# ai4ce/DiscoNet

Measured on AMD Instinct MI355X. Metric: scenes/sec (5-agent 256x256 BEV), higher is better.
Workload: dtype f16 hi+lo pair per value (32 bits; 22-bit significand for |x| >= 0.125, f16 exponent range, lo subnormal below: absolute floor 2^-25); conv products as split-f16 x3 MFMA, f32 accumulate; 1 GPU; DiscoNet det eval forward (--com disco), 5-agent, batch 4 per GPU, 256x256x13 BEV, no KD, sparse voxel lists -> dense -> enc -> DiscoGraph fusion -> dec -> cls/reg heads; agents=5, batch_per_gpu=4, conv_math=sp, launch=hipGraph replay, parallelism=scene-parallel x1 (no data-path collective)

## Files before the change

disconet_amd/csrc/common.hip:

```cpp
#include "dn_internal.h"

namespace dn {
char* err_buf() {
  static thread_local char buf[512] = {0};
  return buf;
}
namespace {
typedef unsigned u32x4 __attribute__((ext_vector_type(4)));
__global__ void __launch_bounds__(256) zero_fill_kernel(unsigned char* p, size_t head, size_t vecs, size_t tail) {
  const size_t tid = blockIdx.x * (size_t)blockDim.x + threadIdx.x, stride = (size_t)gridDim.x * blockDim.x;
  if (tid < head) p[tid] = 0;
  u32x4* v = reinterpret_cast<u32x4*>(p + head);
  for (size_t i = tid; i < vecs; i += stride) v[i] = u32x4{0u, 0u, 0u, 0u};
  if (tid < tail) p[head + 16 * vecs + tid] = 0;
}
}

hipError_t zero_fill(void* ptr, size_t bytes, hipStream_t stream) {
  if (bytes == 0) return hipSuccess;
  unsigned char* p = static_cast<unsigned char*>(ptr);
  size_t head = (16 - (reinterpret_cast<size_t>(p) & 15)) & 15;
  if (head > bytes) head = bytes;
  const size_t vecs = (bytes - head) / 16, tail = bytes - head - 16 * vecs;
  const size_t want = (vecs + 255) / 256;
  const int blocks = (int)(want < 1 ? 1 : (want > 8192 ? 8192 : want));
  hipLaunchKernelGGL(zero_fill_kernel, dim3(blocks), dim3(256), 0, stream, p, head, vecs, tail);
  return hipGetLastError();
}
}

extern "C" int dn_version(void) { return 154; }

#ifndef DN_BUILD_ID
#error "build through disconet_amd/csrc/build.py (it passes -DDN_BUILD_ID)"
#endif
static const char dn_build_id_marker[] = "dn-build-id:" DN_BUILD_ID;
extern "C" const char* dn_build_id(void) { return dn_build_id_marker + 12; }

extern "C" int dn_sp_range_flags_async(unsigned* dst_device, int reset, void* stream) {
  DN_REQUIRE(dst_device != nullptr, "sp_range_flags_async: null destination");
  hipStream_t s = (hipStream_t)stream;
  if ((reset & 2) && dn::zero_fill(dst_device, sizeof(unsigned), s) != hipSuccess)
    return dn::fail(DN_ERR_LAUNCH, "sp_range_flags_async: zero fill of the destination failed");
  const bool clear = (reset & 1) != 0;
  dn::range_collect_conv_sp(dst_device, clear, s);
  dn::range_collect_conv_spq(dst_device, clear, s);
  dn::range_collect_fuse_mlp(dst_device, clear, s);
  dn::range_collect_conv_wgrad(dst_device, clear, s);
  return dn::check_launch("sp_range_collect_kernel");
}

extern "C" unsigned dn_sp_range_flags(int reset) {
  unsigned* d = nullptr;
  unsigned v = 0;
  if (hipDeviceSynchronize() != hipSuccess || hipMalloc((void**)&d, sizeof v) != hipSuccess) return 0x80000000u;
  bool ok = hipMemcpy(d, &v, sizeof v, hipMemcpyHostToDevice) == hipSuccess &&
            dn_sp_range_flags_async(d, reset ? 1 : 0, nullptr) == DN_OK &&
            hipMemcpy(&v, d, sizeof v, hipMemcpyDeviceToHost) == hipSuccess;
  (void)hipFree(d);
  return ok ? v : 0x80000000u;
}

extern "C" const char* dn_last_error(void) { return dn::err_buf(); }
```

disconet_amd/csrc/conv_spq.hip:

```cpp
#ifndef DN_SP_ABL
#define DN_SP_ABL 0
#endif
#include "dn_internal.h"
#include "sp_layout.h"
#include "sp_device.h"
#include "sp_split.h"
#include <type_traits>

namespace {

constexpr int kCUs = 256;

constexpr int QTH = 8, QTW = 32, QPH = QTH + 2, QPW = QTW + 2, QHALF = QPW / 2, QPITCH = QPW, QNPIX = QPH * QPITCH;
constexpr int QNW = 4, QNT = QNW * 64;
constexpr int QA_PIECES = 4 * QNPIX;
constexpr int QA_INSTR = (QA_PIECES + 63) / 64;
constexpr int QA_IT = (QA_INSTR + QNW - 1) / QNW;
constexpr int QA_STAGE = QA_INSTR * 1024;
static_assert(QA_INSTR == 22 && QA_IT == 6, "patch stage: 22 instructions, waves 0 / 1 issue 6, waves 2 / 3 issue 5");

struct SpqArgs {
  const unsigned char* src0;
  const unsigned char* src1;
  const unsigned char* wpk;
  const float* scale;
  const float* shift;
  unsigned char* out;
  float* out_f32;
  int ldo_f32;
  int n_images, h, w;
  int c0g, c1g;
  int c_out, cog, relu;
  int tiles_x, tiles_y, total_items;
  int cout_pad, wpk_bytes;
  int n_cb;
  float rcp_ncb, rcp_tx, rcp_ty;
  KSlices ks;
};

struct QTile {
  int img, oy0, ox0, n0;
};

template <int BN, int DEEP = 0>
struct SpqTile {
  static constexpr int WTN = BN / 32;
  static constexpr int TGQ = DEEP ? 4 : (BN == 64 ? 1 : 2);
  static constexpr int NS0 = 4 / TGQ;
  static constexpr int TG1 = DEEP ? 9 : 3;
  static constexpr int NS1 = 9 / TG1;
  static constexpr int BLK = 4 * BN * 16;
  static constexpr int B_PIECES0 = TGQ * 4 * 4 * BN;
  static constexpr int B_PIECES1 = TG1 * 4 * BN;
  static constexpr int B_IT0 = (B_PIECES0 + QNT - 1) / QNT;
  static constexpr int B_IT1 = (B_PIECES1 + QNT - 1) / QNT;
  static_assert(B_IT1 <= B_IT0, "the source-0 step is the larger one");
  static constexpr int QB_STAGE = B_IT0 * QNT * 16;
  static constexpr int AFF_BYTES = QNW * 2 * 64 * 4;
  static constexpr int LDS_BYTES = 2 * QA_STAGE + 2 * QB_STAGE + AFF_BYTES;
  static_assert((DEEP ? 1 : 2) * LDS_BYTES <= 160 * 1024, "two workgroups per CU (DEEP: one)");
};

template <int BN, int DEEP, int ABL = 0, int KSL = 0>
__global__ void __launch_bounds__(QNT, 2) conv_spq_kernel(const SpqArgs a) {
  static_assert(!KSL || BN == 32, "K slices: the 32-channel tile");
  using T = SpqTile<BN, DEEP>;
  constexpr int WTN = T::WTN, TGQ = T::TGQ, NS0 = T::NS0, NS1 = T::NS1, BLK = T::BLK, QB_STAGE = T::QB_STAGE;
  extern __shared__ __attribute__((aligned(16))) unsigned char smem[];
  constexpr int OFF_B = 2 * QA_STAGE;

  const int tid = threadIdx.x;
  const int lane = tid & 63;
  const int wave = tid >> 6;
  const int li = lane & 31, lh = lane >> 5;
  const int py = wave & 1, px = wave >> 1;

  const int G = gridDim.x;
  const int spatial_items = a.n_images * a.tiles_y * a.tiles_x;
  const int n_cb = a.n_cb;
  const int sp_full = spatial_items & ~7;
  auto decode = [&](int item) {
    QTile tc;
    int cb, spi;
    if (item < sp_full * n_cb) {
      const int j = item >> 3;
      const int jq = fdivmod(j, n_cb, a.rcp_ncb, cb);
      spi = (item & 7) * (sp_full >> 3) + jq;
    } else {
      const int r = item - sp_full * n_cb, rem = spatial_items - sp_full;
      cb = r / rem;
      spi = sp_full + r % rem;
    }
    tc.n0 = cb * BN;
    int tx, ty;
    spi = fdivmod(spi, a.tiles_x, a.rcp_tx, tx);
    tc.img = fdivmod(spi, a.tiles_y, a.rcp_ty, ty);
    tc.ox0 = tx * QTW;
    tc.oy0 = ty * QTH;
    return tc;
  };

  struct Work {
    QTile tc;
    int sl0, sl1, j;
  };
  const int nchunks = a.c0g + a.c1g;
  auto decode_work = [&](int v) {
    Work w;
    if (KSL == 0 || v < a.ks.n_whole) {
      w.tc = decode(v);
      w.sl0 = 0; w.sl1 = KSL ? a.ks.count : 1; w.j = -1;
    } else {
      w.j = v - a.ks.n_whole;
      w.sl0 = w.j & ((1 << a.ks.log2) - 1);
      w.sl1 = w.sl0 + 1;
      w.tc = decode(a.ks.n_whole + (w.j >> a.ks.log2));
    }
    return w;
  };
  auto first_group = [&](const Work& w) { return KSL ? a.ks.bound(w.sl0) : 0; };

  const int rsel = sp::in_g2(li) ? 1 : 0, kcol = sp::rank16(li);
  int prow[2], pcol;
  pcol = px + 2 * kcol;
  auto colpos = [](int e) { return (e & 1) * QHALF + (e >> 1); };
  int a_b1[2][3];
  int a_b0[2][2][2];
#pragma unroll
  for (int wm = 0; wm < 2; ++wm) {
    prow[wm] = py + 4 * wm + 2 * rsel;
#pragma unroll
    for (int dx = 0; dx < 3; ++dx) a_b1[wm][dx] = (lh * QNPIX + prow[wm] * QPITCH + colpos(px + dx) + kcol) * 16;
#pragma unroll
    for (int b = 0; b < 2; ++b)
#pragma unroll
      for (int am = 0; am < 2; ++am)
        a_b0[wm][b][am] = (lh * QNPIX + (prow[wm] + am + (py & am)) * QPITCH + colpos(px + b + (px & b)) + kcol) * 16;
  }
  int b_off[WTN], b_offq[WTN];
#pragma unroll
  for (int wn = 0; wn < WTN; ++wn) {
    b_off[wn] = (lh * BN + wn * 32 + li) * 16;
    b_offq[wn] = b_off[wn] + wave * BLK;
  }

  f32x16 acc[2][WTN];
  f32x16 tot[KSL ? 2 : 1][KSL ? WTN : 1];
  float amax = 0.f;
  bool nan_seen = false;

  constexpr unsigned OOB = 0xFFFFFFFFu;
  const int hs0 = a.h >> 1, ws0 = a.w >> 1;
  const unsigned plane0 = (unsigned)(hs0 * ws0) * 16u, plane1 = (unsigned)(a.h * a.w) * 16u;
  const size_t img0_bytes = (size_t)a.c0g * 4 * plane0, img1_bytes = (size_t)a.c1g * 4 * plane1;
  auto rsrc0 = __builtin_amdgcn_make_buffer_rsrc(const_cast<unsigned char*>(a.src0), 0, 0, 0x00020000);
  auto rsrc1 = rsrc0;
  const auto rsrcw = __builtin_amdgcn_make_buffer_rsrc(const_cast<unsigned char*>(a.wpk), 0, a.wpk_bytes, 0x00020000);
  unsigned voff_a[QA_IT], voff_b[T::B_IT0];

  auto opaque = [](int v) {
    asm volatile("" : "+v"(v));
    return v;
  };
  unsigned piece_map[QA_IT];
#pragma unroll
  for (int it = 0; it < QA_IT; ++it) {
    const int piece = (it * QNW + wave) * 64 + lane;
    const int cq = piece / QNPIX, pp = piece % QNPIX;
    const int r = pp / QPITCH, pos = pp % QPITCH;
    const int cc = pos < QHALF ? 2 * pos : 2 * (pos - QHALF) + 1;
    piece_map[it] = (unsigned)r | ((unsigned)cc << 8) | ((unsigned)cq << 16) | (piece < QA_PIECES ? 0x80000000u : 0u);
  }
  auto setup_voff_a = [&](const QTile& tc, bool from1) {
    const int iy0 = tc.oy0 - 1, ix0 = tc.ox0 - 1;
    const unsigned plane = from1 ? plane1 : plane0;
    const int ws = from1 ? a.w : ws0;
#pragma unroll
    for (int it = 0; it < QA_IT; ++it) {
      unsigned pm = piece_map[it];
      asm volatile("" : "+v"(pm));
      const int r = pm & 0xff, cc = (pm >> 8) & 0xff, cq = (pm >> 16) & 0xff;
      const int iy = iy0 + r, ix = ix0 + cc;
      const bool ok = (int)pm < 0 && iy >= 0 && iy < a.h && ix >= 0 && ix < a.w;
      const int sy = from1 ? iy : (iy >> 1), sx = from1 ? ix : (ix >> 1);
      voff_a[it] = ok ? (unsigned)cq * plane + (unsigned)(sy * ws + sx) * 16u : OOB;
    }
  };
  int voffb_n0 = -1;
  auto setup_voff_b = [&](const QTile& tc) {
    if (tc.n0 == voffb_n0) return;
    voffb_n0 = tc.n0;
    const int t = opaque(tid);
#pragma unroll
    for (int it = 0; it < T::B_IT0; ++it) {
      const int piece = (it * QNW + (t >> 6)) * 64 + (t & 63);
      const int blk = piece / (4 * BN), q = (piece / BN) % 4, nn = piece % BN;
      voff_b[it] = (unsigned)(((blk * 4 + q) * a.cout_pad + tc.n0 + nn) * 16);
    }
  };
  auto setup_rsrc = [&](const QTile& tc) {
    rsrc0 = __builtin_amdgcn_make_buffer_rsrc(const_cast<unsigned char*>(a.src0 + tc.img * img0_bytes), 0,
                                              (int)img0_bytes, 0x00020000);
    rsrc1 = __builtin_amdgcn_make_buffer_rsrc(const_cast<unsigned char*>(a.c1g ? a.src1 + tc.img * img1_bytes : a.src0),
                                              0, a.c1g ? (int)img1_bytes : 0, 0x00020000);
  };
  auto issue_a = [&](int g, int sa) {
    if constexpr ((ABL & 2) != 0) return;
    const bool from1 = g >= a.c0g;
    const int soff = from1 ? (g - a.c0g) * 4 * (int)plane1 : g * 4 * (int)plane0;
    unsigned char* base = smem + sa * QA_STAGE + wave * 1024;
#pragma unroll
    for (int it = 0; it < QA_IT; ++it) {
      if (it == QA_IT - 1 && wave >= QA_INSTR - (QA_IT - 1) * QNW) break;
      if (from1)
        dma16(rsrc1, base + it * QNW * 1024, voff_a[it], soff);
      else
        dma16(rsrc0, base + it * QNW * 1024, voff_a[it], soff);
    }
  };
  auto issue_b = [&](int g, int st, int sb) {
    if constexpr ((ABL & 1) != 0) return;
    const bool from1 = g >= a.c0g;
    const int blk = from1 ? a.c0g * 16 + (g - a.c0g) * 9 + st * T::TG1 : g * 16 + st * (TGQ * 4);
    const int soff = blk * 4 * a.cout_pad * 16;
    unsigned char* base = smem + OFF_B + sb * QB_STAGE + wave * 1024;
#pragma unroll
    for (int it = 0; it < T::B_IT0; ++it)
      if (!from1 || it < T::B_IT1) dma16(rsrcw, base + it * QNW * 1024, voff_b[it], soff);
  };

  struct Frags {
    half8 ah[2], al[2], bh[WTN], bl[WTN];
  };
  auto mma = [&](const Frags& f) {
#pragma unroll
    for (int wm = 0; wm < 2; ++wm)
#pragma unroll
      for (int k = 0; k < WTN; ++k) {
        const int wn = (wm & 1) ? WTN - 1 - k : k;
        acc[wm][wn] = __builtin_amdgcn_mfma_f32_32x32x16_f16(f.bl[wn], f.ah[wm], acc[wm][wn], 0, 0, 0);
      }
#pragma unroll
    for (int wm = 0; wm < 2; ++wm)
#pragma unroll
      for (int k = 0; k < WTN; ++k) {
        const int wn = (wm & 1) ? WTN - 1 - k : k;
        acc[wm][wn] = __builtin_amdgcn_mfma_f32_32x32x16_f16(f.bh[wn], f.al[wm], acc[wm][wn], 0, 0, 0);
      }
#pragma unroll
    for (int wm = 0; wm < 2; ++wm)
#pragma unroll
      for (int k = 0; k < WTN; ++k) {
        const int wn = (wm & 1) ? WTN - 1 - k : k;
        acc[wm][wn] = __builtin_amdgcn_mfma_f32_32x32x16_f16(f.bh[wn], f.ah[wm], acc[wm][wn], 0, 0, 0);
      }
  };
  auto compute1 = [&](auto st_c, const unsigned char* As, const unsigned char* Bs) {
    constexpr int DY = decltype(st_c)::value;
    Frags f[2];
    auto load = [&](auto u_c) {
      constexpr int u = decltype(u_c)::value;
      Frags& d = f[u & 1];
#pragma unroll
      for (int wm = 0; wm < 2; ++wm) {
        d.ah[wm] = *reinterpret_cast<const half8*>(As + a_b1[wm][u] + DY * QPITCH * 16);
        d.al[wm] = *reinterpret_cast<const half8*>(As + a_b1[wm][u] + DY * QPITCH * 16 + 2 * QNPIX * 16);
      }
#pragma unroll
      for (int wn = 0; wn < WTN; ++wn) {
        d.bh[wn] = *reinterpret_cast<const half8*>(Bs + b_off[wn] + u * BLK);
        d.bl[wn] = *reinterpret_cast<const half8*>(Bs + b_off[wn] + u * BLK + 2 * BN * 16);
      }
    };
    load(std::integral_constant<int, 0>{});
    load(std::integral_constant<int, 1>{});
    __builtin_amdgcn_sched_barrier(0);
    mma(f[0]);
    __builtin_amdgcn_sched_barrier(0);
    load(std::integral_constant<int, 2>{});
    __builtin_amdgcn_sched_barrier(0);
    mma(f[1]);
    __builtin_amdgcn_sched_barrier(0);
    mma(f[0]);
    __builtin_amdgcn_sched_barrier(0);
  };
  auto compute0 = [&](auto st_c, const unsigned char* As, const unsigned char* Bs) {
    constexpr int ST = decltype(st_c)::value;
    Frags f[2];
    auto load = [&](auto u_c) {
      constexpr int u = decltype(u_c)::value;
      constexpr int t = ST * TGQ + u, am = t >> 1, b = t & 1;
      Frags& d = f[u & 1];
#pragma unroll
      for (int wm = 0; wm < 2; ++wm) {
        d.ah[wm] = *reinterpret_cast<const half8*>(As + a_b0[wm][b][am]);
        d.al[wm] = *reinterpret_cast<const half8*>(As + a_b0[wm][b][am] + 2 * QNPIX * 16);
      }
#pragma unroll
      for (int wn = 0; wn < WTN; ++wn) {
        d.bh[wn] = *reinterpret_cast<const half8*>(Bs + b_offq[wn] + u * 4 * BLK);
        d.bl[wn] = *reinterpret_cast<const half8*>(Bs + b_offq[wn] + u * 4 * BLK + 2 * BN * 16);
      }
    };
    load(std::integral_constant<int, 0>{});
    if constexpr (TGQ == 4) {
      load(std::integral_constant<int, 1>{});
      __builtin_amdgcn_sched_barrier(0);
      mma(f[0]);
      __builtin_amdgcn_sched_barrier(0);
      load(std::integral_constant<int, 2>{});
      __builtin_amdgcn_sched_barrier(0);
      mma(f[1]);
      __builtin_amdgcn_sched_barrier(0);
      load(std::integral_constant<int, 3>{});
      __builtin_amdgcn_sched_barrier(0);
      mma(f[0]);
      __builtin_amdgcn_sched_barrier(0);
      mma(f[1]);
    } else if constexpr (TGQ == 2) {
      load(std::integral_constant<int, 1>{});
      __builtin_amdgcn_sched_barrier(0);
      mma(f[0]);
      __builtin_amdgcn_sched_barrier(0);
      mma(f[1]);
    } else {
      __builtin_amdgcn_sched_barrier(0);
      mma(f[0]);
    }
    __builtin_amdgcn_sched_barrier(0);
  };

  float* aff_s = reinterpret_cast<float*>(smem + 2 * QA_STAGE + 2 * QB_STAGE) + wave * 128;
  int aff_n0 = -1;
  auto load_affine = [&](int n0) {
    if (n0 == aff_n0) return;
    aff_n0 = n0;
    if (lane < BN) {
      const int co = n0 + lane, ci = min(co, a.c_out - 1);
      aff_s[lane] = co < a.c_out ? a.scale[ci] : 0.f;
      aff_s[64 + lane] = co < a.c_out ? a.shift[ci] : 0.f;
    }
  };
  auto epilogue = [&](const QTile& tc) {
    const int plane = a.h * a.w * 16;
    const int img_bytes = a.cog * 4 * plane;
    const auto rsrc_o = __builtin_amdgcn_make_buffer_rsrc(a.out + (size_t)tc.img * img_bytes, 0, img_bytes, 0x00020000);
    const float lo_clamp = a.relu ? 0.f : -65504.f;
    if (a.out_f32 != nullptr) {
      const float floor_v = a.relu ? 0.f : -__builtin_inff();
#pragma unroll
      for (int wm = 0; wm < 2; ++wm) {
        const int oy = tc.oy0 + prow[wm], ox = tc.ox0 + pcol;
        const bool inside = oy < a.h && ox < a.w;
        float* orow = a.out_f32 + (((size_t)tc.img * a.h + oy) * a.w + ox) * a.ldo_f32;
#pragma unroll
        for (int wn = 0; wn < WTN; ++wn)
#pragma unroll
          for (int g = 0; g < 4; ++g) {
            const int co = tc.n0 + 32 * wn + 8 * g + 4 * lh;
            const f32x4 sc = *reinterpret_cast<const f32x4*>(aff_s + wn * 32 + 8 * g + 4 * lh);
            const f32x4 sh = *reinterpret_cast<const f32x4*>(aff_s + 64 + wn * 32 + 8 * g + 4 * lh);
            f32x4 v = affine4(quad_of(acc[wm][wn], g), sc, sh);
            nan_seen |= !(fabsf(v[0]) <= 3.4028235e38f) | !(fabsf(v[1]) <= 3.4028235e38f) | !(fabsf(v[2]) <= 3.4028235e38f) |
                        !(fabsf(v[3]) <= 3.4028235e38f);
#pragma unroll
            for (int e = 0; e < 4; ++e) v[e] = fmaxf(v[e], floor_v);
            if (inside && co < a.c_out) *reinterpret_cast<f32x4*>(orow + co) = v;
          }
      }
      if (a.out == nullptr) return;
    }
#pragma unroll
    for (int wm = 0; wm < 2; ++wm) {
      const int oy = tc.oy0 + prow[wm], ox = tc.ox0 + pcol;
      const bool inside = oy < a.h && ox < a.w;
      const int voff = inside ? (oy * a.w + ox) * 16 + lh * plane : (int)0x80000000;
#pragma unroll
      for (int wn = 0; wn < WTN; ++wn) {
        u32x2 hi[4], lo[4];
#pragma unroll
        for (int g = 0; g < 4; ++g) {
          const f32x4 sc = *reinterpret_cast<const f32x4*>(aff_s + wn * 32 + 8 * g + 4 * lh);
          const f32x4 sh = *reinterpret_cast<const f32x4*>(aff_s + 64 + wn * 32 + 8 * g + 4 * lh);
          const f32x4 v = affine4(quad_of(acc[wm][wn], g), sc, sh);
          split4(v, hi[g], lo[g], amax, lo_clamp);
        }
#pragma unroll
        for (int m = 0; m < 2; ++m) {
          const u32x4 ph = gather_octet(hi[2 * m], hi[2 * m + 1]);
          const u32x4 pl = gather_octet(lo[2 * m], lo[2 * m + 1]);
          const int cg = (tc.n0 + 32 * wn) / 16 + m;
          if (cg < a.cog) {
            __builtin_amdgcn_raw_buffer_store_b128(ph, rsrc_o, voff + cg * 4 * plane, 0, 0);
            __builtin_amdgcn_raw_buffer_store_b128(pl, rsrc_o, voff + (cg * 4 + 2) * plane, 0, 0);
          }
        }
      }
    }
  };

  int item = blockIdx.x;
  if (item >= a.total_items) return;
  auto partial_of = [&](int j) {
    return a.ks.partial + ((size_t)j * QNW + wave) * (2 * WTN * 16 * 64) + lane * 4;
  };
  auto fold_acc = [&]() {
    if constexpr (KSL != 0) {
#pragma unroll
      for (int wm = 0; wm < 2; ++wm)
#pragma unroll
        for (int wn = 0; wn < WTN; ++wn)
#pragma unroll
          for (int r = 0; r < 16; ++r) {
            tot[wm][wn][r] += acc[wm][wn][r];
            acc[wm][wn][r] = 0.f;
          }
    }
  };
  auto zero_tot = [&]() {
    if constexpr (KSL != 0) {
#pragma unroll
      for (int wm = 0; wm < 2; ++wm)
#pragma unroll
        for (int wn = 0; wn < WTN; ++wn)
#pragma unroll
          for (int r = 0; r < 16; ++r) tot[wm][wn][r] = 0.f;
    }
  };
  auto tot_to_acc = [&]() {
    if constexpr (KSL != 0) {
#pragma unroll
      for (int wm = 0; wm < 2; ++wm)
#pragma unroll
        for (int wn = 0; wn < WTN; ++wn) acc[wm][wn] = tot[wm][wn];
    }
  };
  if constexpr (KSL != 0) {
    if (a.ks.fixup) {
      for (int p = blockIdx.x; p < a.ks.n_split; p += G) {
        const QTile tc = decode(a.ks.n_whole + p);
        load_affine(tc.n0);
        zero_tot();
        for (int sl = 0; sl < a.ks.count; ++sl) {
          const float* pb = partial_of((p << a.ks.log2) + sl);
#pragma unroll
          for (int wm = 0; wm < 2; ++wm)
#pragma unroll
            for (int wn = 0; wn < WTN; ++wn)
#pragma unroll
              for (int q = 0; q < 4; ++q) {
                const f32x4 v = *reinterpret_cast<const f32x4*>(pb + ((wm * WTN + wn) * 4 + q) * 256);
#pragma unroll
                for (int e = 0; e < 4; ++e) acc[wm][wn][4 * q + e] = v[e];
              }
          fold_acc();
        }
        tot_to_acc();
        epilogue(tc);
        note_range(amax, nan_seen);
      }
      return;
    }
  }
  Work cw = decode_work(item);
  QTile cur = cw.tc;
  setup_rsrc(cur);
  setup_voff_b(cur);
  setup_voff_a(cur, first_group(cw) >= a.c0g);
  issue_b(first_group(cw), 0, 0);
  issue_a(first_group(cw), 0);
  int sa = 0, sb = 0;
  bool a_pending = true;

  while (true) {
#pragma unroll
    for (int wm = 0; wm < 2; ++wm)
#pragma unroll
      for (int wn = 0; wn < WTN; ++wn)
#pragma unroll
        for (int r = 0; r < 16; ++r) acc[wm][wn][r] = 0.f;
    load_affine(cur.n0);
    const bool has_next = item + G < a.total_items;
    QTile nxt = cur;
    int ng0 = 0;
    if (has_next) {
      const Work nw = decode_work(item + G);
      nxt = nw.tc;
      ng0 = first_group(nw);
    }
    if constexpr (KSL != 0) zero_tot();
    const int g_end = KSL ? a.ks.bound(cw.sl1) : nchunks;

    for (int sl = cw.sl0; sl < cw.sl1; ++sl) {
    const int g_lo = KSL ? a.ks.bound(sl) : 0, g_hi = KSL ? a.ks.bound(sl + 1) : nchunks;
    for (int g = g_lo; g < g_hi; ++g) {
      const bool last_g = g + 1 == g_end;
      auto step = [&](auto st_c, auto kind_c) {
        constexpr int ST = decltype(st_c)::value;
        constexpr bool SRC1 = decltype(kind_c)::value;
        constexpr int NSG = SRC1 ? NS1 : NS0;
        if (ST == 1 && a_pending) {
          if (wave < QA_INSTR - (QA_IT - 1) * QNW) wait_vm<QA_IT>(); else wait_vm<QA_IT - 1>();
        } else {
          wait_vm0();
        }
        __builtin_amdgcn_s_barrier();
        asm volatile("" ::: "memory");
        if (ST + 1 < NSG) {
          issue_b(g, ST + 1, sb ^ 1);
        } else if (!last_g) {
          issue_b(g + 1, 0, sb ^ 1);
        } else if (has_next) {
          setup_voff_b(nxt);
          issue_b(ng0, 0, sb ^ 1);
        }
        if (ST == 0) {
          a_pending = true;
          if (!last_g) {
            if (g + 1 == a.c0g) setup_voff_a(cur, true);
            issue_a(g + 1, sa ^ 1);
          } else if (has_next) {
            setup_rsrc(nxt);
            setup_voff_a(nxt, ng0 >= a.c0g);
            issue_a(ng0, sa ^ 1);
          } else {
            a_pending = false;
          }
        }
        if constexpr (SRC1 && NS1 == 1) {
          compute1(std::integral_constant<int, 0>{}, smem + sa * QA_STAGE, smem + OFF_B + sb * QB_STAGE);
          compute1(std::integral_constant<int, 1>{}, smem + sa * QA_STAGE, smem + OFF_B + sb * QB_STAGE + 3 * BLK);
          compute1(std::integral_constant<int, 2>{}, smem + sa * QA_STAGE, smem + OFF_B + sb * QB_STAGE + 6 * BLK);
        } else if constexpr (SRC1)
          compute1(st_c, smem + sa * QA_STAGE, smem + OFF_B + sb * QB_STAGE);
        else
          compute0(st_c, smem + sa * QA_STAGE, smem + OFF_B + sb * QB_STAGE);
        sb ^= 1;
      };
      if (g < a.c0g) {
        step(std::integral_constant<int, 0>{}, std::false_type{});
        if constexpr (NS0 >= 2) step(std::integral_constant<int, 1>{}, std::false_type{});
        if constexpr (NS0 == 4) {
          step(std::integral_constant<int, 2>{}, std::false_type{});
          step(std::integral_constant<int, 3>{}, std::false_type{});
        }
      } else {
        step(std::integral_constant<int, 0>{}, std::true_type{});
        if constexpr (NS1 == 3) {
          step(std::integral_constant<int, 1>{}, std::true_type{});
          step(std::integral_constant<int, 2>{}, std::true_type{});
        }
      }
      sa ^= 1;
    }
    if (KSL != 0 && cw.j < 0) fold_acc();
    }
    if (KSL != 0 && cw.j >= 0) {
      if constexpr (KSL != 0) {
        float* pb = partial_of(cw.j);
#pragma unroll
        for (int wm = 0; wm < 2; ++wm)
#pragma unroll
          for (int wn = 0; wn < WTN; ++wn)
#pragma unroll
            for (int q = 0; q < 4; ++q)
              *reinterpret_cast<f32x4*>(pb + ((wm * WTN + wn) * 4 + q) * 256) =
                  f32x4{acc[wm][wn][4 * q], acc[wm][wn][4 * q + 1], acc[wm][wn][4 * q + 2], acc[wm][wn][4 * q + 3]};
      }
    } else {
      tot_to_acc();
      epilogue(cur);
      note_range(amax, nan_seen);
    }
    if (!has_next) break;
    item += G;
    if constexpr (KSL != 0) cw = decode_work(item);
    cur = nxt;
  }
}

__global__ void spq_pack_weights_kernel(const float* __restrict__ w, unsigned char* __restrict__ wpk, int c_out, int c_in,
                                        int c0g, int cout_pad, int nchunks, float wmul) {
  const long total = ((long)c0g * 16 + (long)(nchunks - c0g) * 9) * 2 * cout_pad;
  for (long idx = blockIdx.x * (long)blockDim.x + threadIdx.x; idx < total; idx += (long)gridDim.x * blockDim.x) {
    long r = idx;
    const int n = r % cout_pad; r /= cout_pad;
    const int oct = r % 2; r /= 2;
    int cg, dy0, dy1, dx0, dx1;
    if (r < (long)c0g * 16) {
      cg = (int)(r / 16);
      const int k = (int)(r % 16), t = k / 4, cls = k % 4;
      const int am = t >> 1, b = t & 1, py = cls & 1, px = cls >> 1;
      dy0 = am == 0 ? 0 : (py == 0 ? 1 : 2); dy1 = am == 0 ? (py == 0 ? 0 : 1) : 2;
      dx0 = b == 0 ? 0 : (px == 0 ? 1 : 2);  dx1 = b == 0 ? (px == 0 ? 0 : 1) : 2;
    } else {
      const long q = r - (long)c0g * 16;
      cg = c0g + (int)(q / 9);
      dy0 = dy1 = (int)(q % 9) / 3;
      dx0 = dx1 = (int)(q % 3);
    }
    float v[8];
#pragma unroll
    for (int e = 0; e < 8; ++e) {
      const int ci = cg * 16 + oct * 8 + e;
      v[e] = 0.f;
      if (n < c_out && ci < c_in) {
        const float* wp = w + ((size_t)n * c_in + ci) * 9;
        for (int dy = dy0; dy <= dy1; ++dy)
          for (int dx = dx0; dx <= dx1; ++dx) v[e] += wp[dy * 3 + dx];
        v[e] *= wmul;
      }
    }
    sp::split_store(wpk, sp::weight_piece(r, sp::quarter_of(0, oct), cout_pad, n), (size_t)2 * cout_pad, v);
  }
}

template <int BN, int DEEP = 0, int ABL = 0, int KSL = 0>
int launch_spq(SpqArgs& a, hipStream_t stream, size_t ws_bytes = 0) {
  using T = SpqTile<BN, DEEP>;
  auto kern = conv_spq_kernel<BN, DEEP, ABL, KSL>;
  static dn::PerDeviceFlag attr_flag;
  bool& attr_set = attr_flag.here();
  if (!attr_set) {
    hipError_t e = hipFuncSetAttribute(reinterpret_cast<const void*>(kern), hipFuncAttributeMaxDynamicSharedMemorySize,
                                       (int)T::LDS_BYTES);
    if (e != hipSuccess)
      return dn::fail(DN_ERR_LAUNCH, "spconv (quad-merged): hipFuncSetAttribute(%d B LDS): %s", (int)T::LDS_BYTES,
                      hipGetErrorString(e));
    attr_set = true;
  }
  a.tiles_x = (a.w + QTW - 1) / QTW;
  a.tiles_y = (a.h + QTH - 1) / QTH;
  const long total = (long)a.n_images * a.tiles_y * a.tiles_x * ((a.c_out + BN - 1) / BN);
  DN_REQUIRE(total < (1L << 22), "spconv (quad-merged): too many tiles (%ld)", total);
  DN_REQUIRE((long)a.h * a.w * 16 * 4 * a.cog < (1L << 31), "spconv (quad-merged): one output image exceeds 2 GiB");
  a.total_items = (int)total;
  a.n_cb = (a.c_out + BN - 1) / BN;
  a.rcp_ncb = 1.0f / (float)a.n_cb; a.rcp_tx = 1.0f / (float)a.tiles_x; a.rcp_ty = 1.0f / (float)a.tiles_y;
  const long resident = (DEEP ? 1L : 2L) * kCUs;
  dn::SpLastForm form = {1, 3, 1, QTH, QTW, BN, 0, 1, 0, 0, 2, 0, KSL, 0, DEEP, 0, 0, 0, 0, 0};
  if constexpr (KSL != 0) {
    KSlices& k = a.ks;
    const int S = k.count, ng = a.c0g + a.c1g;
    DN_REQUIRE((S == 2 || S == 4) && ng >= S, "spconv (quad-merged): %d K slices of a %d-chunk layer", S, ng);
    const long wtot = 4L * a.c0g + 9L * a.c1g;
    int b[5] = {0, 0, 0, 0, ng};
    for (int sl = 1; sl < S; ++sl) {
      int g = b[sl - 1] + 1;
      auto before = [&](int gg) { return gg <= a.c0g ? 4L * gg : 4L * a.c0g + 9L * (gg - a.c0g); };
      while (g < ng - (S - 1 - sl) - 1 && before(g) * S < wtot * sl) ++g;
      b[sl] = g;
    }
    k.log2 = S == 4 ? 2 : 1; k.ngroups = ng;
    k.b1 = b[1]; k.b2 = S == 2 ? ng : b[2]; k.b3 = S == 2 ? ng : b[3];
    const size_t per_tile = (size_t)S * QNW * 2 * (BN / 32) * 16 * 64 * sizeof(float);
    k.n_whole = (int)ks_plan(total, resident, S, k.partial ? ws_bytes : 0, per_tile);
    k.n_split = (int)(total - k.n_whole);
    k.fixup = 0;
    const long work = k.n_whole + (long)k.n_split * S;
    a.total_items = (int)work;
    form.grid = (int)(work > resident ? resident : work); form.total_items = (int)work;
    form.n_whole = k.n_whole; form.n_split = k.n_split;
    form.fixup_grid = k.n_split ? (int)(k.n_split > 2 * kCUs ? 2 * kCUs : k.n_split) : 0;
    dn::g_sp_last_form = form;
    hipLaunchKernelGGL(kern, dim3((unsigned)(work > resident ? resident : work)), dim3(QNT), T::LDS_BYTES, stream, a);
    if (k.n_split) {
      k.fixup = 1;
      a.total_items = k.n_split;
      hipLaunchKernelGGL(kern, dim3((unsigned)(k.n_split > 2 * kCUs ? 2 * kCUs : k.n_split)), dim3(QNT), T::LDS_BYTES, stream, a);
    }
    return dn::check_launch("conv_spq_kernel (K slices)");
  }
  dim3 grid((unsigned)(total > resident ? resident : total));
  form.grid = (int)grid.x; form.total_items = (int)total; form.n_whole = (int)total;
  dn::g_sp_last_form = form;
  hipLaunchKernelGGL(kern, grid, dim3(QNT), T::LDS_BYTES, stream, a);
  return dn::check_launch("conv_spq_kernel");
}

}

namespace dn {

void range_collect_conv_spq(unsigned* dst, bool reset, hipStream_t s) { sp_range_collect_here(dst, reset, s); }

size_t spq_packed_blocks(int c0g, int nchunks) { return (size_t)c0g * 16 + (size_t)(nchunks - c0g) * 9; }

int spq_pack_weights(const float* weight_oihw, void* packed, int c_out, int c_in, int c0g, int cout_pad, int nchunks,
                     float wmul, hipStream_t stream) {
  hipLaunchKernelGGL(spq_pack_weights_kernel, dim3(2048), dim3(256), 0, stream, weight_oihw, (unsigned char*)packed, c_out,
                     c_in, c0g, cout_pad, nchunks, wmul);
  return check_launch("spq_pack_weights_kernel");
}

int spq_conv(const dn_conv_desc* d, const void* src0, const void* src1, const void* packed, size_t packed_bytes,
             const float* scale, const float* shift, void* out, int cout_pad, int bn, hipStream_t stream,
             int kslices, float* workspace, size_t workspace_bytes, float* out_nhwc, int ld_nhwc) {
  SpqArgs a;
  a.src0 = (const unsigned char*)src0; a.src1 = (const unsigned char*)src1; a.wpk = (const unsigned char*)packed;
  a.scale = scale; a.shift = shift; a.out = (unsigned char*)out;
  a.out_f32 = out_nhwc; a.ldo_f32 = ld_nhwc;
  a.n_images = d->n_images; a.h = d->h_in; a.w = d->w_in;
  a.c0g = (d->c0 + 15) / 16; a.c1g = (d->c1 + 15) / 16;
  a.c_out = d->c_out; a.cog = (d->c_out + 15) / 16; a.relu = d->relu;
  a.cout_pad = cout_pad; a.wpk_bytes = (int)packed_bytes;
  a.tiles_x = a.tiles_y = a.total_items = 0;
  a.ks = KSlices{workspace, kslices, 0, 0, 0, 0, 0, 0, 0, 0};
  if (kslices > 1) {
    const long tiles = (long)d->n_images * ((d->h_in + QTH - 1) / QTH) * ((d->w_in + QTW - 1) / QTW);
    const bool deep = tiles * ((d->c_out + 31) / 32) * kslices <= (long)kCUs;
    if (bn == 33 || (bn == 0 && deep)) return launch_spq<32, 1, 0, 1>(a, stream, workspace_bytes);
    return launch_spq<32, 0, 0, 1>(a, stream, workspace_bytes);
  }
  if (bn == 0) {
    const long tiles = (long)d->n_images * ((d->h_in + QTH - 1) / QTH) * ((d->w_in + QTW - 1) / QTW);
    bn = (d->c_out > 32 && tiles * ((d->c_out + 63) / 64) >= 4L * kCUs) ? 64 : 32;
    if (bn == 32 && tiles * ((d->c_out + 31) / 32) <= (long)kCUs) bn = 33;
  }
  if (bn == 64) return launch_spq<64>(a, stream);
  if (bn == 33) return launch_spq<32, 1>(a, stream);
#if DN_SP_ABL
  if (bn == 101) return launch_spq<32, 0, 1>(a, stream);
  if (bn == 102) return launch_spq<32, 0, 2>(a, stream);
  if (bn == 103) return launch_spq<32, 0, 3>(a, stream);
#endif
  return launch_spq<32>(a, stream);
}

}
```

Baseline: 2298 scenes/s.

## Regroup source-1 taps into fewer steps and drop per-step barriers on wave-local weights

New measurement: 2302 scenes/s (median of 2 runs). Within noise of the previous version (+0.2%).

```diff
diff --git a/disconet_amd/csrc/common.hip b/disconet_amd/csrc/common.hip
--- a/disconet_amd/csrc/common.hip
+++ b/disconet_amd/csrc/common.hip
@@ -29,7 +29,7 @@
 }
 }
 
-extern "C" int dn_version(void) { return 154; }
+extern "C" int dn_version(void) { return 155; }
 
 #ifndef DN_BUILD_ID
 #error "build through disconet_amd/csrc/build.py (it passes -DDN_BUILD_ID)"
diff --git a/disconet_amd/csrc/conv_spq.hip b/disconet_amd/csrc/conv_spq.hip
--- a/disconet_amd/csrc/conv_spq.hip
+++ b/disconet_amd/csrc/conv_spq.hip
@@ -10,6 +10,8 @@
 namespace {
 
 constexpr int kCUs = 256;
+
+__device__ inline void wait_lgkm0() { asm volatile("s_waitcnt lgkmcnt(0)" ::: "memory"); }
 
 constexpr int QTH = 8, QTW = 32, QPH = QTH + 2, QPW = QTW + 2, QHALF = QPW / 2, QPITCH = QPW, QNPIX = QPH * QPITCH;
 constexpr int QNW = 4, QNT = QNW * 64;
@@ -47,15 +49,15 @@
   static constexpr int WTN = BN / 32;
   static constexpr int TGQ = DEEP ? 4 : (BN == 64 ? 1 : 2);
   static constexpr int NS0 = 4 / TGQ;
-  static constexpr int TG1 = DEEP ? 9 : 3;
-  static constexpr int NS1 = 9 / TG1;
+  static constexpr int NS1 = DEEP ? 1 : (BN == 32 ? 2 : 3);
+  static constexpr int tap1_lo(int st) { return DEEP ? 0 : (BN == 32 ? 5 * st : 3 * st); }
+  static constexpr int tap1_n(int st) { return DEEP ? 9 : (BN == 32 ? (st == 0 ? 5 : 4) : 3); }
   static constexpr int BLK = 4 * BN * 16;
-  static constexpr int B_PIECES0 = TGQ * 4 * 4 * BN;
-  static constexpr int B_PIECES1 = TG1 * 4 * BN;
-  static constexpr int B_IT0 = (B_PIECES0 + QNT - 1) / QNT;
-  static constexpr int B_IT1 = (B_PIECES1 + QNT - 1) / QNT;
-  static_assert(B_IT1 <= B_IT0, "the source-0 step is the larger one");
-  static constexpr int QB_STAGE = B_IT0 * QNT * 16;
+  static constexpr int IPB = BLK / 1024;
+  static constexpr int NBLK = TGQ * 4;
+  static constexpr int B_IT = TGQ * IPB;
+  static_assert(tap1_n(0) <= NBLK, "the source-0 step is the larger one");
+  static constexpr int QB_STAGE = NBLK * BLK;
   static constexpr int AFF_BYTES = QNW * 2 * 64 * 4;
   static constexpr int LDS_BYTES = 2 * QA_STAGE + 2 * QB_STAGE + AFF_BYTES;
   static_assert((DEEP ? 1 : 2) * LDS_BYTES <= 160 * 1024, "two workgroups per CU (DEEP: one)");
@@ -156,7 +158,7 @@
   auto rsrc0 = __builtin_amdgcn_make_buffer_rsrc(const_cast<unsigned char*>(a.src0), 0, 0, 0x00020000);
   auto rsrc1 = rsrc0;
   const auto rsrcw = __builtin_amdgcn_make_buffer_rsrc(const_cast<unsigned char*>(a.wpk), 0, a.wpk_bytes, 0x00020000);
-  unsigned voff_a[QA_IT], voff_b[T::B_IT0];
+  unsigned voff_a[QA_IT], voff_b[T::B_IT];
 
   auto opaque = [](int v) {
     asm volatile("" : "+v"(v));
@@ -192,9 +194,9 @@
     voffb_n0 = tc.n0;
     const int t = opaque(tid);
 #pragma unroll
-    for (int it = 0; it < T::B_IT0; ++it) {
-      const int piece = (it * QNW + (t >> 6)) * 64 + (t & 63);
-      const int blk = piece / (4 * BN), q = (piece / BN) % 4, nn = piece % BN;
+    for (int it = 0; it < T::B_IT; ++it) {
+      const int piece = (it % T::IPB) * 64 + (t & 63);
+      const int blk = (it / T::IPB) * 4 + (t >> 6), q = piece / BN, nn = piece % BN;
       voff_b[it] = (unsigned)(((blk * 4 + q) * a.cout_pad + tc.n0 + nn) * 16);
     }
   };
@@ -221,12 +223,16 @@
   auto issue_b = [&](int g, int st, int sb) {
     if constexpr ((ABL & 1) != 0) return;
     const bool from1 = g >= a.c0g;
-    const int blk = from1 ? a.c0g * 16 + (g - a.c0g) * 9 + st * T::TG1 : g * 16 + st * (TGQ * 4);
+    const int nblk = from1 ? T::tap1_n(st) : T::NBLK;
+    const int blk = from1 ? a.c0g * 16 + (g - a.c0g) * 9 + T::tap1_lo(st) : g * 16 + st * T::NBLK;
     const int soff = blk * 4 * a.cout_pad * 16;
-    unsigned char* base = smem + OFF_B + sb * QB_STAGE + wave * 1024;
-#pragma unroll
-    for (int it = 0; it < T::B_IT0; ++it)
-      if (!from1 || it < T::B_IT1) dma16(rsrcw, base + it * QNW * 1024, voff_b[it], soff);
+    unsigned char* base = smem + OFF_B + sb * QB_STAGE + wave * BLK;
+#pragma unroll
+    for (int u = 0; u < TGQ; ++u) {
+      if (u * 4 + wave >= nblk) break;
+#pragma unroll
+      for (int i = 0; i < T::IPB; ++i) dma16(rsrcw, base + u * 4 * BLK + i * 1024, voff_b[u * T::IPB + i], soff);
+    }
   };
 
   struct Frags {
@@ -255,21 +261,22 @@
         acc[wm][wn] = __builtin_amdgcn_mfma_f32_32x32x16_f16(f.bh[wn], f.ah[wm], acc[wm][wn], 0, 0, 0);
       }
   };
-  auto compute1 = [&](auto st_c, const unsigned char* As, const unsigned char* Bs) {
-    constexpr int DY = decltype(st_c)::value;
+  auto compute1 = [&](auto t0_c, auto nt_c, const unsigned char* As, const unsigned char* Bs) {
+    constexpr int T0 = decltype(t0_c)::value, NT = decltype(nt_c)::value;
+    static_assert(NT >= 3 && NT <= 5 && T0 + NT <= 9, "taps of one step");
     Frags f[2];
-    auto load = [&](auto u_c) {
-      constexpr int u = decltype(u_c)::value;
-      Frags& d = f[u & 1];
+    auto load = [&](auto i_c) {
+      constexpr int i = decltype(i_c)::value, DY = (T0 + i) / 3, DX = (T0 + i) % 3;
+      Frags& d = f[i & 1];
 #pragma unroll
       for (int wm = 0; wm < 2; ++wm) {
-        d.ah[wm] = *reinterpret_cast<const half8*>(As + a_b1[wm][u] + DY * QPITCH * 16);
-        d.al[wm] = *reinterpret_cast<const half8*>(As + a_b1[wm][u] + DY * QPITCH * 16 + 2 * QNPIX * 16);
+        d.ah[wm] = *reinterpret_cast<const half8*>(As + a_b1[wm][DX] + DY * QPITCH * 16);
+        d.al[wm] = *reinterpret_cast<const half8*>(As + a_b1[wm][DX] + DY * QPITCH * 16 + 2 * QNPIX * 16);
       }
 #pragma unroll
       for (int wn = 0; wn < WTN; ++wn) {
-        d.bh[wn] = *reinterpret_cast<const half8*>(Bs + b_off[wn] + u * BLK);
-        d.bl[wn] = *reinterpret_cast<const half8*>(Bs + b_off[wn] + u * BLK + 2 * BN * 16);
+        d.bh[wn] = *reinterpret_cast<const half8*>(Bs + b_off[wn] + i * BLK);
+        d.bl[wn] = *reinterpret_cast<const half8*>(Bs + b_off[wn] + i * BLK + 2 * BN * 16);
       }
     };
     load(std::integral_constant<int, 0>{});
@@ -281,8 +288,24 @@
     __builtin_amdgcn_sched_barrier(0);
     mma(f[1]);
     __builtin_amdgcn_sched_barrier(0);
+    if constexpr (NT > 3) {
+      load(std::integral_constant<int, 3>{});
+      __builtin_amdgcn_sched_barrier(0);
+    }
     mma(f[0]);
     __builtin_amdgcn_sched_barrier(0);
+    if constexpr (NT > 4) {
+      load(std::integral_constant<int, 4>{});
+      __builtin_amdgcn_sched_barrier(0);
+    }
+    if constexpr (NT > 3) {
+      mma(f[1]);
+      __builtin_amdgcn_sched_barrier(0);
+    }
+    if constexpr (NT > 4) {
+      mma(f[0]);
+      __builtin_amdgcn_sched_barrier(0);
+    }
   };
   auto compute0 = [&](auto st_c, const unsigned char* As, const unsigned char* Bs) {
     constexpr int ST = decltype(st_c)::value;
@@ -504,7 +527,11 @@
         } else {
           wait_vm0();
         }
-        __builtin_amdgcn_s_barrier();
+        constexpr bool MEET = ST == 0 || SRC1;
+        if constexpr (MEET)
+          __builtin_amdgcn_s_barrier();
+        else
+          wait_lgkm0();
         asm volatile("" ::: "memory");
         if (ST + 1 < NSG) {
           issue_b(g, ST + 1, sb ^ 1);
@@ -527,12 +554,14 @@
             a_pending = false;
           }
         }
+        [[maybe_unused]] constexpr std::integral_constant<int, 3> three{};
         if constexpr (SRC1 && NS1 == 1) {
-          compute1(std::integral_constant<int, 0>{}, smem + sa * QA_STAGE, smem + OFF_B + sb * QB_STAGE);
-          compute1(std::integral_constant<int, 1>{}, smem + sa * QA_STAGE, smem + OFF_B + sb * QB_STAGE + 3 * BLK);
-          compute1(std::integral_constant<int, 2>{}, smem + sa * QA_STAGE, smem + OFF_B + sb * QB_STAGE + 6 * BLK);
+          compute1(std::integral_constant<int, 0>{}, three, smem + sa * QA_STAGE, smem + OFF_B + sb * QB_STAGE);
+          compute1(std::integral_constant<int, 3>{}, three, smem + sa * QA_STAGE, smem + OFF_B + sb * QB_STAGE + 3 * BLK);
+          compute1(std::integral_constant<int, 6>{}, three, smem + sa * QA_STAGE, smem + OFF_B + sb * QB_STAGE + 6 * BLK);
         } else if constexpr (SRC1)
-          compute1(st_c, smem + sa * QA_STAGE, smem + OFF_B + sb * QB_STAGE);
+          compute1(std::integral_constant<int, T::tap1_lo(ST)>{}, std::integral_constant<int, T::tap1_n(ST)>{},
+                   smem + sa * QA_STAGE, smem + OFF_B + sb * QB_STAGE);
         else
           compute0(st_c, smem + sa * QA_STAGE, smem + OFF_B + sb * QB_STAGE);
         sb ^= 1;
@@ -546,10 +575,8 @@
         }
       } else {
         step(std::integral_constant<int, 0>{}, std::true_type{});
-        if constexpr (NS1 == 3) {
-          step(std::integral_constant<int, 1>{}, std::true_type{});
-          step(std::integral_constant<int, 2>{}, std::true_type{});
-        }
+        if constexpr (NS1 >= 2) step(std::integral_constant<int, 1>{}, std::true_type{});
+        if constexpr (NS1 == 3) step(std::integral_constant<int, 2>{}, std::true_type{});
       }
       sa ^= 1;
     }
```
